# CWBudde/go-pocket-tts

Hardware: AMD Instinct MI355X
Metric: synthesized audio sec/sec (xRT) (higher is better)
Workload: dtype bf16; 1 GPU; b64_10s_bf16: 64 utterances/GPU x 125 frames (10.0 s each), 25-token prompt + 125-frame voice state, greedy (temperature 0), hipGraph-captured AR step, Mimi decode to 24 kHz PCM written to host; batch_per_gpu=64, frames=125, weights=BF16, kv=bf16, checkpoint=synthetic, shapes of tts_b6369a24 (seed 1234)

## Files before the change

### go-pocket-tts_amd/csrc/capi_hooks.cpp

```cpp
#include "capi_internal.h"
#include "launch_args.h"
#include "../../include/ptts_debug.h"
#include "scan_block.h"
#include "true_peak.h"

#include <memory>

using namespace ptts;
using namespace ptts::capi;

namespace {

template <class T> class Scoped {
    T& var_;
    T old_;
public:
    Scoped(T& var, T value) : var_(var), old_(var) { var = value; }
    ~Scoped() { var_ = old_; }
    Scoped(const Scoped&) = delete;
    Scoped& operator=(const Scoped&) = delete;
};

using Census = std::map<std::string, int64_t>;

// ... 1159 lines not shown
        if (t.ls) up(dLs.as<float>() + t.ls_off, t.ls, (size_t)D * 4);
        if (rope) { up(dCos.p, t.rope_cos, ntab * 4); up(dSin.p, t.rope_sin, ntab * 4); }
        LaunchScope launches;
        launches.run([&] {
            if (ffn) launch_mimi_ffn(fa, nullptr);
            else launch_mimi_rowlin(ra, nullptr);
        });
        PTTS_HIP(hipGetLastError());
        PTTS_HIP(hipDeviceSynchronize());
        put_str(t.launched, t.launched_cap, launches.str());
        if (ffn) down(t.out, dX.p, (size_t)t.x_elems * 4);
        else down(t.out, dY, (size_t)t.y_elems * 4);
    });
}

int ptts_mimi_layer_piece(ptts_model* h, int32_t layer, int32_t which, const float* x, int64_t rows, int32_t pos0, int32_t rows_per_seg, float* out) {
    return guard([&] {
        if (!h || !h->m) throw Error(PTTS_EINVAL, "native-safetensors runtime unavailable");
        Model& m = *h->m;
        const Desc& d = m.d;
        if (!x || !out || rows <= 0 || rows > (1 << 24)) throw Error(PTTS_EINVAL, "ptts-hip: bad rows");
        if (layer < 0 || layer >= d.mimi_layers) throw Error(PTTS_EINVAL, strfmt("ptts-hip: mimi layer %d out of range [0,%d)", layer, d.mimi_layers));
        if (which != PTTS_MIMI_PIECE_QKV && which != PTTS_MIMI_PIECE_FFN) throw Error(PTTS_EINVAL, "ptts-hip: unknown layer piece");
        if (pos0 < 0 || rows_per_seg < 0 || (int64_t)pos0 + (rows_per_seg ? rows_per_seg : rows) > ROPE_SEQ)
            throw Error(PTTS_EINVAL, strfmt("ops: rope cos/sin sequence length too small for pos=%d seq=%lld", pos0, (long long)(rows_per_seg ? rows_per_seg : rows)));
        std::lock_guard<std::mutex> lock(m.mu);
        m.use_device();
        const int C = d.mimi_dim, F = d.mimi_ffn, R = (int)rows;
        const int NO = which == PTTS_MIMI_PIECE_QKV ? 3 * C : C;
        Tmp dx((size_t)R * C * 4), dn((size_t)R * C * 4), dy((size_t)R * std::max(NO, F) * 4);
// ... 14 lines not shown
```

### go-pocket-tts_amd/csrc/ffn_fused.hip

```cpp
#include <cstdlib>
#include <type_traits>

#include "kernels.h"
#include "device_util.h"
#include "mfma_util.h"

namespace ptts {

namespace {

__device__ __forceinline__ float ff_gelu(float x) {
    const float ax = fabsf(x);
    const float t = __builtin_amdgcn_rcpf(fmaf(0.3275911f * 0.70710678118654752f, ax, 1.0f));
    float p = fmaf(1.061405429f, t, -1.453152027f);
    p = fmaf(p, t, 1.421413741f);
    p = fmaf(p, t, -0.284496736f);
    p = fmaf(p, t, 0.254829592f);
    p *= t;
    const float e = __builtin_amdgcn_exp2f(-1.4426950408889634f * 0.5f * x * x);
    const float erfa = fmaf(-p, e, 1.0f);
    const float erfs = copysignf(erfa, x);
    return 0.5f * x * (1.0f + erfs);
}

// ... 42 lines not shown
    for (int s = 0; s < 16; s++) {
        float4 o[2];
#pragma unroll
        for (int h = 0; h < 2; h++) {
            const int k = 32 * s + 16 * h + 4 * q;
            const float4 g = *reinterpret_cast<const float4*>(ln_w + k), b = *reinterpret_cast<const float4*>(ln_b + k);
            o[h].x = (v[s][h].x - mean) * rstd * g.x + b.x;
            o[h].y = (v[s][h].y - mean) * rstd * g.y + b.y;
            o[h].z = (v[s][h].z - mean) * rstd * g.z + b.z;
            o[h].w = (v[s][h].w - mean) * rstd * g.w + b.w;
        }
        split2(o[0].x, o[0].y, xh[s].u[0], xl[s].u[0]);
        split2(o[0].z, o[0].w, xh[s].u[1], xl[s].u[1]);
        split2(o[1].x, o[1].y, xh[s].u[2], xl[s].u[2]);
        split2(o[1].z, o[1].w, xh[s].u[3], xl[s].u[3]);
    }
}

template <class Piece>
__device__ __forceinline__ void ff_gemm1(const char* w1, int r16, int q, const Frag (&xh)[16], const Frag (&xl)[16], f32x4 (&acc)[2], Piece&& piece) {
    const int sw1 = (r16 >> 1) & 7;
    acc[0] = f32x4{0.f, 0.f, 0.f, 0.f};
    acc[1] = f32x4{0.f, 0.f, 0.f, 0.f};
    Frag wa[2], wb[2];
    const char* wl = w1 + r16 * 128;
    wa[0].q = *reinterpret_cast<const uint4*>(wl + ((q ^ sw1) << 4));
    wb[0].q = *reinterpret_cast<const uint4*>(wl + ((q ^ sw1) << 4) + 2048);
#pragma unroll
    for (int s = 0; s < 16; s++) {
        __builtin_amdgcn_sched_barrier(0);
// ... 104 lines not shown
#pragma unroll
            for (int t = 0; t < 8; t++) {
#pragma clang fp contract(off)
                const f32x4 y = acc2[t0 + t];
                float4 o;
                o.x = r[t].x + sc[t].x * y[0];
                o.y = r[t].y + sc[t].y * y[1];
                o.z = r[t].z + sc[t].z * y[2];
                o.w = r[t].w + sc[t].w * y[3];
                *reinterpret_cast<float4*>(orow + 16 * (t0 + t) + 4 * q) = o;
            }
        }
    }
}

__global__ __launch_bounds__(256) __attribute__((amdgpu_waves_per_eu(1, 1))) void k_mimi_rowlin(RowLinArgs a) {
    constexpr int NS = 3;
    __shared__ __attribute__((aligned(16))) char lds[NS * FF_W1B];
    const int tid = threadIdx.x, lane = tid & 63, wave = __builtin_amdgcn_readfirstlane(tid >> 6);
    const int r16 = lane & 15, q = lane >> 4;
    const int nch = a.N / FF_CH;
    const char* img = reinterpret_cast<const char*>(a.img);
    ff_dma32k(img, lds, wave, lane);
    ff_dma32k(img + (size_t)min(1, nch - 1) * FF_W1B, lds + FF_W1B, wave, lane);

    const int m0 = blockIdx.x * 64 + wave * 16;
    const int row = min(m0 + r16, a.M - 1);
    Frag xh[FF_KS], xl[FF_KS];
    ff_rows_layernorm(a.x + row_off(a.xmap, row), a.ln_w, a.ln_b, a.eps, q, xh, xl);
    float2 cs[4], sn[4];
    const bool rope = a.rope_cos != nullptr;
    {
        const int pos = a.rope_pos0 + (a.rope_rows_per_seg ? row % a.rope_rows_per_seg : row);
        const float* ct = rope ? a.rope_cos + (int64_t)pos * 32 : a.ln_w;
        const float* st = rope ? a.rope_sin + (int64_t)pos * 32 : a.ln_w;
#pragma unroll
        for (int i = 0; i < 4; i++) {
            const int jj = (32 * (i >> 1) + 16 * (i & 1) + 4 * q) >> 1;
            cs[i] = *reinterpret_cast<const float2*>(ct + jj);
            sn[i] = *reinterpret_cast<const float2*>(st + jj);
        }
    }
    float* const yrow = a.y + row_off(a.ymap, row);

    auto store_piece = [&](f32x4 (&acc)[2], int cc, auto par, int ht) {
#pragma clang fp contract(off)
        constexpr int PAR = decltype(par)::value;
        asm volatile("" : "+a"(acc[0]), "+a"(acc[1]));
        const int col = 32 * cc + 16 * ht + 4 * q;
        const bool rot = rope && 32 * cc < a.rope_cols;
        const f32x4 v = acc[ht];
        const float2 c2 = cs[2 * PAR + ht], s2 = sn[2 * PAR + ht];
        const float y0 = v[0] * c2.x - v[1] * s2.x, y1 = v[0] * s2.x + v[1] * c2.x;
        const float y2 = v[2] * c2.y - v[3] * s2.y, y3 = v[2] * s2.y + v[3] * c2.y;
        const float4 o = make_float4(rot ? y0 : v[0], rot ? y1 : v[1], rot ? y2 : v[2], rot ? y3 : v[3]);
        *reinterpret_cast<float4*>(yrow + col) = o;
    };

    asm volatile("s_waitcnt vmcnt(0)" ::: "memory");
    __syncthreads();
    f32x4 accA[2], accB[2];
    auto iter = [&](int c, auto par, auto first, f32x4 (&acc)[2], f32x4 (&prev)[2]) {
        constexpr int PAR = decltype(par)::value;
        constexpr bool FIRST = decltype(first)::value != 0;
        if constexpr (!FIRST) {
            asm volatile("s_waitcnt vmcnt(10)" ::: "memory");
            __syncthreads();
        }
        const char* const src = img + (size_t)min(c + 2, nch - 1) * FF_W1B + wave * 1024 + lane * 16;
        char* const dst = lds + ((c + 2) % NS) * FF_W1B + wave * 1024;
        ff_gemm1(lds + (c % NS) * FF_W1B, r16, q, xh, xl, acc, [&](int s) {
            if ((s & 1) == 0) lds_dma1k(src + (s >> 1) * 4096, dst + (s >> 1) * 4096);
            if constexpr (!FIRST) {
                if (s == 5) store_piece(prev, c - 1, std::integral_constant<int, 1 - PAR>{}, 0);
                if (s == 11) store_piece(prev, c - 1, std::integral_constant<int, 1 - PAR>{}, 1);
            }
        });
    };
    using ic0 = std::integral_constant<int, 0>;
    using ic1 = std::integral_constant<int, 1>;
    iter(0, ic0{}, ic1{}, accA, accB);
    iter(1, ic1{}, ic0{}, accB, accA);
    for (int c = 2; c < nch; c += 2) {
        iter(c, ic0{}, ic0{}, accA, accB);
        iter(c + 1, ic1{}, ic0{}, accB, accA);
    }
    store_piece(accB, nch - 1, std::integral_constant<int, 1>{}, 0);
    store_piece(accB, nch - 1, std::integral_constant<int, 1>{}, 1);
}

bool mimi_rowlin_supported(const RowLinArgs& a) {
    return a.img && a.K == FF_D && a.N >= 64 && a.N % 64 == 0 && a.M > 0 && aligned16(a.x) && a.xmap.ld % 4 == 0 && a.xmap.batch_stride % 4 == 0 && aligned16(a.y) &&
           a.ymap.ld % 4 == 0 && a.ymap.batch_stride % 4 == 0 && aligned16(a.img) && a.ln_w && a.ln_b && aligned16(a.ln_w) && aligned16(a.ln_b) &&
           (!a.rope_cos || (a.rope_sin && a.rope_cols % 64 == 0 && a.rope_cols <= a.N && (reinterpret_cast<uintptr_t>(a.rope_cos) & 7) == 0 && (reinterpret_cast<uintptr_t>(a.rope_sin) & 7) == 0));
}

void launch_mimi_rowlin(const RowLinArgs& a, hipStream_t stream) {
    note_launch(a.rope_cos ? "k_mimi_rowlin+rope" : "k_mimi_rowlin");
    hipLaunchKernelGGL(k_mimi_rowlin, dim3((unsigned)((a.M + 63) / 64)), dim3(256), 0, stream, a);
}

bool mimi_ffn_supported(const FfnArgs& a) {
    return a.img && a.D == FF_D && a.F >= FF_CH && a.F % FF_CH == 0 && a.M > 0 && aligned16(a.x) && a.xmap.ld % 4 == 0 && a.xmap.batch_stride % 4 == 0 &&
           aligned16(a.img) && a.ln_w && a.ln_b && aligned16(a.ln_w) && aligned16(a.ln_b) && (!a.ls || aligned16(a.ls));
}

void launch_mimi_ffn(const FfnArgs& a, hipStream_t stream) {
    note_launch("k_mimi_ffn");
    const dim3 grid((unsigned)((a.M + 63) / 64));
    hipLaunchKernelGGL(k_mimi_ffn<0>, grid, dim3(256), 0, stream, a);
}

}
```

### go-pocket-tts_amd/csrc/kernels.h

```cpp
#pragma once

#include <hip/hip_runtime.h>
#include <atomic>
#include <cstddef>
#include <cstdint>
#include <map>
#include <string>
#include <vector>

#include "deesser.h"
#include "limiter.h"
#include "pitch.h"
#include "tempo.h"
#include "trim.h"

namespace ptts {

struct RowMap {
    int64_t ld = 0;
    int64_t rows_per_batch = 0;
    int64_t batch_stride = 0;
};

enum AOp : int { AOP_NONE = 0, AOP_ELU = 1 };
// ... 398 lines not shown

struct FfnArgs {
    float* x = nullptr; RowMap xmap;
    const float* ln_w = nullptr; const float* ln_b = nullptr; float eps = 1e-5f;
    const void* img = nullptr;
    const float* ls = nullptr;
    int M = 0, D = 0, F = 0;
};
struct RowLinArgs {
    const float* x = nullptr; RowMap xmap;
    const float* ln_w = nullptr; const float* ln_b = nullptr; float eps = 1e-5f;
    const void* img = nullptr;
    float* y = nullptr; RowMap ymap;
    const float* rope_cos = nullptr; const float* rope_sin = nullptr; int rope_cols = 0, rope_pos0 = 0, rope_rows_per_seg = 0;
    int M = 0, N = 0, K = 0;
};
bool mimi_rowlin_supported(const RowLinArgs& a);
void launch_mimi_rowlin(const RowLinArgs& a, hipStream_t stream);
bool mimi_ffn_supported(const FfnArgs& a);
void launch_mimi_ffn(const FfnArgs& a, hipStream_t stream);

constexpr int FC_MAX_DEPTH = 8;
struct FlowClusterArgs {
    const float* fx_in = nullptr; float* fx_out = nullptr;
    const float* ada = nullptr; int64_t ldmod = 0;
    int rows = 0, depth = 0;
    float eps[FC_MAX_DEPTH] = {};
    const float* ln_w[FC_MAX_DEPTH] = {}; const float* ln_b[FC_MAX_DEPTH] = {};
    const void* w0[FC_MAX_DEPTH] = {}; const float* b0[FC_MAX_DEPTH] = {};
    const void* w2[FC_MAX_DEPTH] = {}; const float* b2[FC_MAX_DEPTH] = {};
    unsigned long long* xbuf = nullptr;
    unsigned long long* stamps = nullptr;
    int inject = 0;
// ... 68 lines not shown
```

### go-pocket-tts_amd/csrc/mimi_decode.cpp

```cpp
#include "launch_args.h"

#include <algorithm>

namespace ptts {

void mimi_setup(Model& m, MimiWs& w, int B, int T) {
    const Desc& d = m.d;
    w.B = B; w.T = T;
    const int C = d.mimi_dim, S = d.up_stride, T1 = T * S, F = d.mimi_ffn;
    w.P0 = d.init_k - 1;
    w.Ls[0] = T1; w.Ps[0] = 1;
    for (int j = 0; j < 3; j++) {
        w.Ls[j + 1] = w.Ls[j] * d.strides[j];
        int need_next = j < 2 ? 1 : d.final_k - 1;
        w.Ps[j + 1] = std::max(d.rb_k1[j] - 1, need_next);
    }
    size_t n_xp = (size_t)B * (1 + T) * C, n_up = (size_t)B * (w.P0 + T1) * C;
    size_t n_n1 = (size_t)B * T1 * C, n_qkv = (size_t)B * T1 * 3 * C, n_ff = (size_t)B * T1 * F;
    size_t n_c[4], n_h[3];
    for (int j = 0; j < 4; j++) n_c[j] = (size_t)B * (w.Ps[j] + w.Ls[j]) * d.sea_ch[j];
    for (int j = 0; j < 3; j++) n_h[j] = (size_t)B * ((d.rb_k2[j] - 1) + w.Ls[j + 1]) * d.sea_hidden[j];
    size_t total = n_xp + n_up + n_n1 + n_qkv * d.mimi_layers + n_n1 + n_ff + n_c[0] + 2 * (n_c[1] + n_c[2] + n_c[3]) + n_h[0] + n_h[1] + n_h[2];
    DevBuf& wsb = m.work(WORK_DECODER, total * sizeof(float));
    float* p = wsb.as<float>();
// ... 39 lines not shown
        ra.M = R; ra.N = 3 * C; ra.K = C;
        if (mimi_rowlin_supported(ra)) { launch_mimi_rowlin(ra, s); return; }
    }
    launch_layernorm(mkln(m, x, xmap, L.n1, n1, C, R), s);
    GemmArgs gq = mk(m, n1, flat(C), L.in_proj, qkv, qmap, R);
    gq.rope_cos = m.at<float>(d.rope_cos); gq.rope_sin = m.at<float>(d.rope_sin);
    gq.rope_cols = 2 * C; gq.rope_hd = d.mimi_hd; gq.rope_pos0 = pos0; gq.rope_rows_per_seg = rows_per_seg;
    if (!launch_gemm_rope(gq, s)) {
        gq.rope_cos = gq.rope_sin = nullptr;
        launch_gemm(gq, s);
        launch_rope_rows(qkv, qmap, 0, d.mimi_heads, d.mimi_hd, nullptr, pos0, rows_per_seg, R, m.at<float>(d.rope_cos), m.at<float>(d.rope_sin), s);
        launch_rope_rows(qkv, qmap, C, d.mimi_heads, d.mimi_hd, nullptr, pos0, rows_per_seg, R, m.at<float>(d.rope_cos), m.at<float>(d.rope_sin), s);
    }
}

void mimi_layer_ffn(Model& m, int l, float* x, RowMap xmap, int R, float* n1, float* ffb, hipStream_t s) {
    mimi_layer_ffn(m, m.d.ml[l], x, xmap, R, n1, ffb, s);
}
void mimi_layer_ffn(Model& m, const Desc::ML& L, float* x, RowMap xmap, int R, float* n1, float* ffb, hipStream_t s) {
    const Desc& d = m.d;
    const int C = d.mimi_dim, F = d.mimi_ffn;
    if (L.ffn_img != NONE) {
        FfnArgs fa;
        fa.x = x; fa.xmap = xmap;
        fa.ln_w = m.at<float>(L.n2.w); fa.ln_b = m.at<float>(L.n2.b); fa.eps = L.n2.eps;
        fa.img = m.at<uint8_t>(L.ffn_img);
        fa.ls = m.at<float>(L.ls2);
        fa.M = R; fa.D = C; fa.F = F;
        if (mimi_ffn_supported(fa)) { launch_mimi_ffn(fa, s); return; }
    }
// ... 13 lines not shown
    const int B = w.B, T = w.T, C = d.mimi_dim, S = d.up_stride, T1 = T * S, P0 = w.P0;
    if (f1 <= f0) return;
    if (!w.zeroed) mimi_zero_history(m, w, s);
    const int nf = f1 - f0;
    launch_projector(lat, lat_bstride, m.at<float>(d.proj_w), m.at<float>(d.proj_b), B, T, f0, f1, d.ldim, C, w.xp, s);
    if (mimi_latent) launch_btc_to_bct(w.xp, 1, B, C, T, mimi_latent, s);
    launch_upsample_depthwise(w.xp, m.at<float>(d.up_w0), m.at<float>(d.up_w1), nullptr, B, T, f0, f1, C, S, w.up, P0, s);
    const int t0 = f0 * S, CT = nf * S, R = B * CT;
    const int64_t up_bs = (int64_t)(P0 + T1) * C;
    float* upx = w.up + (size_t)(P0 + t0) * C;
    const RowMap upm = seg(C, CT, up_bs);
    float* n1 = w.n1;
    float* attn = w.attn;
    float* ffb = w.ff;
    for (int l = 0; l < d.mimi_layers; l++) {
        const auto& L = d.ml[l];
        float* qkv = w.qkv[l];
        float* qkvx = qkv + (size_t)t0 * 3 * C;
        const RowMap qm = seg(3 * C, CT, (int64_t)T1 * 3 * C);
        mimi_layer_qkv(m, l, upx, upm, R, qkvx, qm, t0, CT, n1, s);
        launch_attention(attn_dense_args(qkv, 3 * C, C, B, T1, t0, CT, d.mimi_heads, d.mimi_hd, d.mimi_ctx, attn, C), s);
        GemmArgs go = mk(m, attn, flat(C), L.out_proj, upx, upm, R);
        go.R = upx; go.epi = L.ls1 != NONE ? EPI_SCALE_RESADD : EPI_RESADD; go.scale = m.at<float>(L.ls1);
        launch_gemm(go, s);
        mimi_layer_ffn(m, l, upx, upm, R, n1, ffb, s);
    }
    if (xformer_out)
        PTTS_HIP(hipMemcpy2DAsync(xformer_out + (size_t)t0 * C, (size_t)T1 * C * sizeof(float), upx, (size_t)up_bs * sizeof(float), (size_t)CT * C * sizeof(float),
                                  (size_t)B, hipMemcpyDeviceToDevice, s));
    int r0 = t0, rn = CT;
    {
        const int ch = d.sea_ch[0];
        GemmArgs g = mk(m, w.up + (size_t)r0 * C, seg(C, rn, up_bs), d.init_conv, w.c0 + (size_t)(w.Ps[0] + r0) * ch,
                        seg(ch, rn, (int64_t)(w.Ps[0] + w.Ls[0]) * ch), B * rn);
        g.epi = EPI_ELU;
        if (C % 64 == 0 && d.init_conv.in == d.init_k * C) { g.win_taps = d.init_k; g.win_c = C; }
        launch_gemm(g, s);
    }
    bool final_done = false;
// ... 91 lines not shown
```

### go-pocket-tts_amd/csrc/runtime.cpp

```cpp
#include "launch_args.h"

#include <chrono>

#include <algorithm>

namespace ptts {

static thread_local UploadArena* tl_upload = nullptr;
static void arena_open(UploadArena& a) {
    if (!a.base && hipHostMalloc((void**)&a.base, (size_t)1 << 20, hipHostMallocDefault) == hipSuccess) a.cap = (size_t)1 << 20;
    else if (!a.base) (void)hipGetLastError();
    a.off = 0;
    tl_upload = &a;
}
UploadScope::UploadScope(UploadArena& a, hipStream_t s) {
    (void)hipStreamSynchronize(s);
    arena_open(a);
}
UploadScope::UploadScope(UploadArena& a, hipEvent_t last_use) {
    if (last_use) (void)hipEventSynchronize(last_use);
    arena_open(a);
}
UploadScope::~UploadScope() { tl_upload = nullptr; }
void h2d(void* dst, const void* src, size_t bytes, hipStream_t s) {
// ... 14 lines not shown
    if (!bytes) return;
    PTTS_HIP(hipMemcpyAsync(dst, src, bytes, hipMemcpyDeviceToHost, s));
    PTTS_HIP(hipStreamSynchronize(s));
}

Model::~Model() {
    if (upload.base) (void)hipHostFree(upload.base);
    for (hipEvent_t e : prof.ev) (void)hipEventDestroy(e);
    for (hipEvent_t e : prof.phase) if (e) (void)hipEventDestroy(e);
    for (hipEvent_t e : events) (void)hipEventDestroy(e);
    if (stream2) (void)hipStreamDestroy(stream2);

    cached_batch.reset();
    tcomb.clear();
    for (DevBuf& w : ws) w.release();
    if (own_arena && arena) (void)hipFree(arena);
    if (stream) (void)hipStreamDestroy(stream);
}

static std::unique_ptr<Model> model_on(const Desc& d, const ptts_opts& opts, int device) {
    std::unique_ptr<Model> m(new Model());
    m->d = d;
    m->opts = opts;
    m->opts.device = m->device = device;
    m->noise_state = (uint64_t)std::chrono::system_clock::now().time_since_epoch().count() ^ (uint64_t)(uintptr_t)m.get();
    return m;
}
static void open_streams(Model& m) {
    m.use_device();
    int lo = 0, hi = 0;
// ... 12 lines not shown
    open_streams(*m);
    if (device_arena) {
        m->arena = reinterpret_cast<uint8_t*>(device_arena);
    } else {
        void* p = nullptr;
        PTTS_HIP(hipMalloc(&p, m->d.total_bytes));
        m->arena = reinterpret_cast<uint8_t*>(p);
        m->own_arena = true;
        fill = 1;
    }
    if (fill) {
        std::vector<uint8_t> host(m->d.total_bytes, 0);
        plan_fill(*plan, host.data());
        PTTS_HIP(hipMemcpy(m->arena, host.data(), host.size(), hipMemcpyHostToDevice));
    }
    return m.release();
}

Model* model_share(Model& base) {
    std::unique_ptr<Model> m = model_on(base.d, base.opts, base.device);
    open_streams(*m);
    m->arena = base.arena;
    m->own_arena = false;
    return m.release();
}

Model* model_replicate(Model& base, int device) {
    int ndev = 0;
    if (hipGetDeviceCount(&ndev) != hipSuccess || ndev <= 0) throw Error(PTTS_ENODEVICE, "ptts-hip: no HIP device available (this library has no CPU fallback)");
    if (device < 0 || device >= ndev) throw Error(PTTS_ENODEVICE, strfmt("ptts-hip: device %d out of range (%d visible)", device, ndev));
    std::unique_ptr<Model> m = model_on(base.d, base.opts, device);
    {
        std::lock_guard<std::mutex> lock(base.mu);
        base.use_device();
        PTTS_HIP(hipStreamSynchronize(base.stream));
    }
    open_streams(*m);
    void* p = nullptr;
    PTTS_HIP(hipMalloc(&p, m->d.total_bytes));
    m->arena = reinterpret_cast<uint8_t*>(p);
    m->own_arena = true;
    if (device != base.device) {
        int can = 0;
        if (hipDeviceCanAccessPeer(&can, device, base.device) == hipSuccess && can) {
            const hipError_t e = hipDeviceEnablePeerAccess(base.device, 0);
            if (e != hipSuccess && e != hipErrorPeerAccessAlreadyEnabled) (void)hipGetLastError();
            else if (e == hipErrorPeerAccessAlreadyEnabled) (void)hipGetLastError();
        }
    }
    PTTS_HIP(hipMemcpyPeer(m->arena, device, base.arena, base.device, m->d.total_bytes));
    PTTS_HIP(hipDeviceSynchronize());
    return m.release();
}

void profile_read(Model& m, ptts_profile* out) {
    PTTS_HIP(hipStreamSynchronize(m.stream));
    std::memset(out, 0, sizeof *out);
    double ms = 0;
    for (size_t i = 0; i + 1 < m.prof.used; i += 2) {
        float t = 0;
        PTTS_HIP(hipEventElapsedTime(&t, m.prof.ev[i], m.prof.ev[i + 1]));
        ms += t;
    }
    out->launches = m.prof.launches;
    out->total_ms = ms;
    out->algorithmic_bytes = m.prof.bytes;
// ... 107 lines not shown
```

### go-pocket-tts_amd/csrc/runtime.h

```cpp
#pragma once

#include <atomic>
#include <functional>
#include <type_traits>

#include "kernels.h"
#include "model.h"
#include "row_ring.h"
#include "dsp_spec.h"
#include "host_rows.h"
#include "join.h"

namespace ptts {

struct DevBuf {
    void* p = nullptr;
    size_t n = 0;
    DevBuf() = default;
    DevBuf(const DevBuf&) = delete;
    DevBuf& operator=(const DevBuf&) = delete;
    ~DevBuf() { release(); }
    void release() {
        if (p) (void)hipFree(p);
        p = nullptr;
// ... 126 lines not shown
    size_t cap = 0, off = 0;
};

struct Model {
    Desc d;
    ptts_opts opts;
    uint8_t* arena = nullptr;
    bool own_arena = false;
    int device = 0;
    hipStream_t stream = nullptr;
    hipStream_t stream2 = nullptr;
    std::vector<hipEvent_t> events;
    std::mutex mu;
    std::map<int, std::unique_ptr<DevBuf>> tcomb;
    DevBuf ws[kWorkSlots];
    std::unique_ptr<Batch> cached_batch;
    Prof prof;
    std::map<std::pair<int, int>, std::unique_ptr<RateFilter>> rate_filters;
    RowRing<ResampleRow> rs_ring;
    RowRing<CmpRow, kCmpMaxDesigns * kCmpScanBytes> cmp_ring;
    RowRing<LimRow, kLimMaxDesigns * kLimScanBytes> lim_ring;
    RowRing<DeRow, kDeMaxDesigns * kDeScanBytes> de_ring;
    RowRing<JoinRow> join_ring;
    RowRing<JoinGainRow> join_gain_ring;
    RowRing<TrimRow, kTrimMaxDesigns * kTrimScanBytes> trim_ring;
    RowRing<TempoRow, kTempoMaxDesigns * kTempoScanBytes> tempo_ring;
    RowRing<PitchRow, kPitchMaxDesigns * kPitchScanBytes> pitch_ring;
    std::unique_ptr<UploadedTable> pitch_image;
    RowRing<FormantRow> formant_ring;
    std::unique_ptr<UploadedTable> formant_tables;
// ... 105 lines not shown

struct MimiWs {
    int B = 0, T = 0, P0 = 0;
    int Ls[4] = {0, 0, 0, 0}, Ps[4] = {0, 0, 0, 0};
    float *xp = nullptr, *up = nullptr, *n1 = nullptr, *qkv[MAX_LAYERS] = {nullptr}, *attn = nullptr, *ff = nullptr, *c0 = nullptr;
    float *u[3] = {nullptr, nullptr, nullptr}, *uo[3] = {nullptr, nullptr, nullptr}, *h[3] = {nullptr, nullptr, nullptr};
    bool zeroed = false;
};
constexpr int kMimiGroup = 64;
void mimi_setup(Model& m, MimiWs& w, int B, int T);
void mimi_range(Model& m, MimiWs& w, const float* lat, int64_t lat_bstride, int f0, int f1, float* pcm, float* mimi_latent, hipStream_t s,
                const PcmRow* pcm_rows = nullptr, bool* rows_used = nullptr, float* xformer_out = nullptr);

void mimi_layer_qkv(Model& m, int layer, const float* x, RowMap xmap, int R, float* qkv, RowMap qmap, int pos0, int rows_per_seg, float* n1, hipStream_t s);
void mimi_layer_ffn(Model& m, int layer, float* x, RowMap xmap, int R, float* n1, float* ffb, hipStream_t s);
void mimi_layer_qkv(Model& m, const Desc::ML& L, const float* x, RowMap xmap, int R, float* qkv, RowMap qmap, int pos0, int rows_per_seg, float* n1, hipStream_t s);
void mimi_layer_ffn(Model& m, const Desc::ML& L, float* x, RowMap xmap, int R, float* n1, float* ffb, hipStream_t s);

constexpr int kEncStages = 10;
int64_t mimi_encode_max_frames(const Desc& d);
void mimi_encode(Model& m, const float* const* pcm, const int64_t* n_samples, int n_clips, float* const* latent_out, float* const* stages = nullptr,
                 const int32_t* rates = nullptr);
int64_t mimi_encode_clip(Model& m, const float* pcm, int64_t n_samples, float* lat_dev, float* const* stages = nullptr, int rate = kNativeRate);
int64_t mimi_encode_samples(int64_t n_samples, int rate);
void require_encoder(const Desc& d);
void mimi_encode_stage_shapes(const Desc& d, int64_t n_samples, int64_t* shapes );
Model* model_open(Plan* plan, void* device_arena, int fill);
void profile_read(Model& m, ptts_profile* out);
Batch* batch_new(Model& m, int n_slots, int cap, int max_steps);
void batch_reset(Batch& b);
// ... 192 lines not shown
```

### go-pocket-tts_amd/runtime.py

```python
from __future__ import annotations

import ctypes as C
import os
import subprocess
import sys
from dataclasses import dataclass, field
from typing import Callable, Optional, Sequence

import numpy as np

_HERE = os.path.dirname(os.path.abspath(__file__))
LIB_PATH = os.environ.get("PTTS_LIB_PATH") or os.path.join(_HERE, "libptts_hip.so")

PTTS_OK, PTTS_EINVAL, PTTS_EIO, PTTS_EFORMAT, PTTS_ENODEVICE, PTTS_ECANCELLED, PTTS_ENOMEM = range(7)
WEIGHTS_F32, WEIGHTS_BF16, WEIGHTS_INT8 = 0, 1, 2
KV_F32, KV_BF16 = 0, 1
PCM_F32, PCM_S16, PCM_ULAW, PCM_ALAW = 0, 1, 2, 3
_PCM_DTYPES = {PCM_F32: "<f4", PCM_S16: "<i2", PCM_ULAW: "|u1", PCM_ALAW: "|u1"}

_FP = C.POINTER(C.c_float)
_IP = C.POINTER(C.c_int64)
_DP = C.POINTER(C.c_double)
_I32P = C.POINTER(C.c_int32)
_STEP_CB = C.CFUNCTYPE(None, C.c_void_p, C.c_int32, C.c_int32)
# ... 218 lines not shown
    "ptts_join_parts_length", "ptts_join_parts", "ptts_join_parts_rows", "ptts_join_parts_stream_ready", "ptts_generate_joined_parts",
    "ptts_trim_plan", "ptts_trim_apply", "ptts_trim_rows", "ptts_dsp_ext_set_trim",
    "ptts_tempo_length", "ptts_tempo_plan", "ptts_tempo_apply", "ptts_tempo_rows", "ptts_dsp_ext_set_tempo",
    "ptts_pitch_speed", "ptts_pitch_resample_length", "ptts_pitch_resample", "ptts_pitch_length", "ptts_pitch_apply", "ptts_pitch_table",
    "ptts_pitch_rows", "ptts_dsp_ext_set_pitch",
    "ptts_formant_frames", "ptts_formant_analyse", "ptts_formant_whiten", "ptts_formant_shape", "ptts_formant_apply", "ptts_formant_rows",
    "ptts_dsp_ext_set_formant",
    ]
HOOK_SYMBOLS = [
    "ptts_decode_stages", "ptts_mimi_layer_piece", "ptts_debug_last_attention_kernel", "ptts_debug_launch_counts", "ptts_debug_flow_cluster_inject",
    "ptts_debug_time_skinny", "ptts_debug_skinny_stamps", "ptts_debug_gemm", "ptts_debug_step_stamps", "ptts_debug_tall_linear",
    "ptts_debug_encode_stages", "ptts_debug_resample_launches", "ptts_debug_dsp_blocked_host",
    "ptts_debug_loudness_energies", "ptts_debug_kweighting", "ptts_debug_step_linear", "ptts_debug_true_peak_taps", "ptts_debug_true_peak_oversample",
    "ptts_debug_dsp_opts_error", "ptts_debug_resblock", "ptts_debug_resblock_plan", "ptts_debug_seanet_pack", "ptts_debug_plan_seanet_frags",
    "ptts_debug_gemm_rows", "ptts_debug_attn_step", "ptts_debug_attn_step_rounds", "ptts_debug_attn_window", "ptts_debug_flow_cluster",
    "ptts_debug_mimi_fused", "ptts_debug_mimi_pack", "ptts_debug_dsp_windows", "ptts_debug_step_edge",
]


def build(force: bool = False) -> str:
    args = ["make", "-s", "-C", _HERE, "-j8"]
    if force:
        args.append("-B")
    subprocess.check_call(args)
    return LIB_PATH


def lib():
    global _lib
    if _lib is None:
        if not os.path.exists(LIB_PATH):
# ... 1469 lines not shown
    a.y_ld, a.y_rows_per_batch, a.y_batch_stride, a.y_off = (int(v) for v in ymap)
    a.x, a.ln_w, a.ln_b, a.w1, a.w2, a.ls = ptr(x_buf), ptr(ln_w), ptr(ln_b), ptr(w1), ptr(w2), ptr(ls)
    if rope is not None:
        cos, sin = (None if t is None else _f32(t) for t in rope)
        a.rope_cos, a.rope_sin = ptr(cos), ptr(sin)
        a.n_pos = (cos if cos is not None else sin).shape[0]
        a.rope_cols, a.pos0, a.rows_per_seg = int(rope_cols), int(pos0), int(rows_per_seg)
    out = np.empty(x_buf.size if int(kind) == 0 else max(int(y_elems), 1), np.float32)
    a.out = ptr(out)
    name = C.create_string_buffer(512)
    a.launched, a.launched_cap = C.cast(name, C.c_char_p), 512
    _check(hooks().ptts_debug_mimi_fused(C.byref(a)))
    return {"out": out, "launched": _census_dict(name)}


def debug_mimi_pack(kind, w1, w2=None):
    w1 = _f32(w1)
    n = w1.shape[0]
    if w1.ndim != 2 or w1.shape[1] != 512 or (kind == 0 and (w2 is None or tuple(np.shape(w2)) != (512, n))):
        raise ValueError("w1 is [n, 512], w2 [512, n]")
    w2 = None if kind != 0 else _f32(w2)
    dst = np.empty(n * (1024 if kind == 0 else 512), np.uint16)
    H = hooks()
    H.ptts_debug_mimi_pack.argtypes = [C.c_int32, _FP, _FP, C.c_int32, C.c_void_p]
    _check(H.ptts_debug_mimi_pack(int(kind), _fp(w1), C.cast(None, _FP) if w2 is None else _fp(w2), n, dst.ctypes.data_as(C.c_void_p)))
    return dst.reshape((n // 32, 2, 16384) if kind == 0 else (n // 32, 16384))


class _ResblockArgs(C.Structure):
    _fields_ = ([(n, C.c_int32) for n in ("B", "L", "t0", "t1", "C", "H", "pad", "slack", "w_bf16", "final_conv", "form", "grid", "fuse_up", "x_pad", "x_L", "x_slack")] +
# ... 878 lines not shown
```

### include/ptts_debug.h

```cpp
#ifndef PTTS_DEBUG_H
#define PTTS_DEBUG_H

#include "ptts.h"

#ifdef __cplusplus
extern "C" {
#endif

#define PTTS_MIMI_PIECE_QKV 0
#define PTTS_MIMI_PIECE_FFN 1
int  ptts_mimi_layer_piece(ptts_model* m, int32_t layer, int32_t which, const float* x, int64_t rows, int32_t pos0, int32_t rows_per_seg, float* out);

int  ptts_decode_stages(ptts_model* m, const float* latents, int32_t n_utt, int32_t frames,
                        float* pcm, float* mimi_latent, float* transformer_out);

int  ptts_debug_encode_stages(ptts_model* m, const float* pcm, int64_t n_samples, float* const* stages, int64_t* shapes);

int ptts_debug_time_skinny(int32_t M, int32_t N, int32_t K, int32_t w_bf16, int32_t splitk, int32_t fuse_ln, int32_t iters, float* avg_us);
int ptts_debug_skinny_stamps(int32_t M, int32_t N, int32_t K, int32_t w_bf16, int32_t splitk, int32_t fuse_ln, uint64_t* out ,
                             int32_t max_blocks, int32_t* n_blocks);
int ptts_debug_step_stamps(ptts_batch* b, int32_t lsd_steps, uint64_t* out , int64_t cap_blocks, int32_t* desc ,
                           int32_t cap_desc, int32_t* n_desc);
int ptts_debug_gemm(int32_t M, int32_t N, int32_t K, int32_t w_bf16, int32_t variant, int32_t epi, int32_t iters, float* avg_us,
                    float* maxdiff);
// ... 115 lines not shown
    char* launched;
} ptts_flow_cluster_args;
int ptts_debug_flow_cluster(const ptts_flow_cluster_args* a);

typedef struct ptts_mimi_fused_args {
    int32_t kind, M, D, F, n_pos, rope_cols, pos0, rows_per_seg, ls_off, reserved;
    float eps, reserved_f;
    int64_t x_elems, x_ld, x_rows_per_batch, x_batch_stride, x_off, y_elems, y_ld, y_rows_per_batch, y_batch_stride, y_off, launched_cap;
    const float *x, *ln_w, *ln_b, *w1, *w2, *ls, *rope_cos, *rope_sin;
    float* out;
    char* launched;
} ptts_mimi_fused_args;
int ptts_debug_mimi_fused(const ptts_mimi_fused_args* a);
int ptts_debug_mimi_pack(int32_t kind, const float* w1, const float* w2, int32_t n, uint16_t* dst);

int64_t ptts_debug_dsp_opts_error(const ptts_dsp_opts* opts, char* out, int64_t cap);
int ptts_debug_true_peak_taps(float* out , int32_t* L, int32_t* K, int32_t* dlo);
int ptts_debug_true_peak_oversample(const float* samples, int64_t n, float* y );

#ifdef __cplusplus
}
#endif
#endif
```

Measured before the change: 12890 x real-time.

## Route Mimi attention out-projection through pre-packed row-linear kernel with residual epilogue

Adds a residual-add variant of the k_mimi_rowlin kernel, templated on the epilogue. The Mimi transformer's 512x512 attention output projection now uses it instead of the generic GEMM. Weight images in the swizzled LDS-DMA layout are packed once at model load, and the kernel skips layernorm and rope, applying the layer-scale and residual add in its epilogue. The aim is to replace a generic GEMM with the tuned, pipelined weight-streaming kernel. The cost is extra device memory for the packed images, plus a load-time pack and sync.

After: 12850 x real-time. No clear change (-0.3%).

```diff
diff --git a/go-pocket-tts_amd/csrc/capi_hooks.cpp b/go-pocket-tts_amd/csrc/capi_hooks.cpp
--- a/go-pocket-tts_amd/csrc/capi_hooks.cpp
+++ b/go-pocket-tts_amd/csrc/capi_hooks.cpp
@@ -1197,6 +1197,48 @@
     });
 }
 
+int ptts_debug_mimi_out(const ptts_mimi_out_args* pa) {
+    return guard([&] {
+        if (!pa) throw Error(PTTS_EINVAL, "ptts_debug_mimi_out: null argument");
+        const ptts_mimi_out_args& t = *pa;
+        constexpr int D = 512;
+        if (!t.attn || !t.r || !t.w || !t.out || t.M < 1 || t.M > (1 << 20) || t.attn_rows < t.M || t.x_elems < 1 || t.x_ld < 1 || t.x_rows_per_batch < 0 ||
+            t.x_rows_per_batch > INT32_MAX || t.x_batch_stride < 0 || t.x_off < 0 || (t.w_bf16 | t.path | t.in_place) & ~1)
+            throw Error(PTTS_EINVAL, "ptts_debug_mimi_out: bad arguments");
+        if (t.x_ld % 4 || t.x_batch_stride % 4 || t.x_off % 4) throw Error(PTTS_EINVAL, "ptts_debug_mimi_out: x_ld, x_batch_stride and x_off must be multiples of 4");
+        const RowMap xmap{t.x_ld, t.x_rows_per_batch, t.x_batch_stride};
+        check_rows("ptts_debug_mimi_out", "r", t.M, t.x_elems, xmap, t.x_off, D, true);
+        require_device();
+        Stage st;
+        const size_t nw = (size_t)D * D;
+        GemmArgs go;
+        const uint8_t* img = nullptr;
+        if (t.w_bf16) {
+            std::vector<uint16_t> w16(nw);
+            for (size_t i = 0; i < nw; i++) w16[i] = f32_to_bf16_rne(t.w[i]);
+            go.W = st.in(w16.data(), nw);
+            if (t.path == 0) {
+                uint16_t* dimg = st.out<uint16_t>(nw);
+                launch_w1_image_pack(go.W, dimg, D, nullptr);
+                img = reinterpret_cast<const uint8_t*>(dimg);
+            }
+        } else go.W = st.in(t.w, nw);
+        go.w_bf16 = t.w_bf16; go.ldw = D;
+        go.A = st.in(t.attn, (size_t)t.attn_rows * D); go.amap = flat(D);
+        float* const dR = st.in(t.r, (size_t)t.x_elems);
+        float* const dY = t.in_place ? dR : st.out((size_t)t.x_elems);
+        go.R = dR + t.x_off; go.C = dY + t.x_off; go.cmap = xmap;
+        go.scale = st.in(t.ls, (size_t)D); go.epi = t.ls ? EPI_SCALE_RESADD : EPI_RESADD;
+        go.M = t.M; go.N = D; go.K = D;
+        LaunchScope launches;
+        launches.run([&] { mimi_out_launch(go, img, nullptr); });
+        PTTS_HIP(hipGetLastError());
+        PTTS_HIP(hipDeviceSynchronize());
+        put_str(t.launched, t.launched_cap, launches.str());
+        down(t.out, dY, (size_t)t.x_elems * 4);
+    });
+}
+
 int ptts_mimi_layer_piece(ptts_model* h, int32_t layer, int32_t which, const float* x, int64_t rows, int32_t pos0, int32_t rows_per_seg, float* out) {
     return guard([&] {
         if (!h || !h->m) throw Error(PTTS_EINVAL, "native-safetensors runtime unavailable");
diff --git a/go-pocket-tts_amd/csrc/ffn_fused.hip b/go-pocket-tts_amd/csrc/ffn_fused.hip
--- a/go-pocket-tts_amd/csrc/ffn_fused.hip
+++ b/go-pocket-tts_amd/csrc/ffn_fused.hip
@@ -80,6 +80,22 @@
         split2(o[0].z, o[0].w, xh[s].u[1], xl[s].u[1]);
         split2(o[1].x, o[1].y, xh[s].u[2], xl[s].u[2]);
         split2(o[1].z, o[1].w, xh[s].u[3], xl[s].u[3]);
+    }
+}
+
+__device__ __forceinline__ void ff_rows_split(const float* xrow, int q, Frag (&xh)[16], Frag (&xl)[16]) {
+    float4 v[16][2];
+#pragma unroll
+    for (int s = 0; s < 16; s++) {
+        v[s][0] = *reinterpret_cast<const float4*>(xrow + 32 * s + 4 * q);
+        v[s][1] = *reinterpret_cast<const float4*>(xrow + 32 * s + 16 + 4 * q);
+    }
+#pragma unroll
+    for (int s = 0; s < 16; s++) {
+        split2(v[s][0].x, v[s][0].y, xh[s].u[0], xl[s].u[0]);
+        split2(v[s][0].z, v[s][0].w, xh[s].u[1], xl[s].u[1]);
+        split2(v[s][1].x, v[s][1].y, xh[s].u[2], xl[s].u[2]);
+        split2(v[s][1].z, v[s][1].w, xh[s].u[3], xl[s].u[3]);
     }
 }
 
@@ -214,23 +230,42 @@
     }
 }
 
+template <int EPI>
 __global__ __launch_bounds__(256) __attribute__((amdgpu_waves_per_eu(1, 1))) void k_mimi_rowlin(RowLinArgs a) {
+    constexpr bool RES = EPI == ROWLIN_RESADD;
     constexpr int NS = 3;
-    __shared__ __attribute__((aligned(16))) char lds[NS * FF_W1B];
+    __shared__ __attribute__((aligned(16))) char lds[NS * FF_W1B + (RES ? FF_D * 4 : 0)];
     const int tid = threadIdx.x, lane = tid & 63, wave = __builtin_amdgcn_readfirstlane(tid >> 6);
     const int r16 = lane & 15, q = lane >> 4;
-    const int nch = a.N / FF_CH;
+    const int nch = RES ? FF_D / FF_CH : a.N / FF_CH;
     const char* img = reinterpret_cast<const char*>(a.img);
     ff_dma32k(img, lds, wave, lane);
     ff_dma32k(img + (size_t)min(1, nch - 1) * FF_W1B, lds + FF_W1B, wave, lane);
 
     const int m0 = blockIdx.x * 64 + wave * 16;
     const int row = min(m0 + r16, a.M - 1);
+    const bool live = m0 + r16 < a.M;
+    const float* const xrow = a.x + row_off(a.xmap, row);
+    float* const yrow = a.y + row_off(a.ymap, row);
     Frag xh[FF_KS], xl[FF_KS];
-    ff_rows_layernorm(a.x + row_off(a.xmap, row), a.ln_w, a.ln_b, a.eps, q, xh, xl);
+    float4 rr[RES ? FF_OT : 1];
+    const float* const lsl = reinterpret_cast<const float*>(lds + NS * FF_W1B);
+    if constexpr (RES) {
+        float2 sv = make_float2(1.f, 1.f);
+        if (a.ls) sv = *reinterpret_cast<const float2*>(a.ls + 2 * tid);
+        *reinterpret_cast<float2*>(lds + NS * FF_W1B + 8 * tid) = sv;
+        const float* const rrow = live ? a.res + row_off(a.ymap, row) : xrow;
+#pragma unroll
+        for (int t = 0; t < FF_OT; t++) rr[t] = *reinterpret_cast<const float4*>(rrow + 16 * t + 4 * q);
+        ff_rows_split(xrow, q, xh, xl);
+#pragma unroll
+        for (int t = 0; t < FF_OT; t++) asm volatile("" : "+v"(rr[t].x), "+v"(rr[t].y), "+v"(rr[t].z), "+v"(rr[t].w));
+    } else {
+        ff_rows_layernorm(xrow, a.ln_w, a.ln_b, a.eps, q, xh, xl);
+    }
     float2 cs[4], sn[4];
-    const bool rope = a.rope_cos != nullptr;
-    {
+    const bool rope = !RES && a.rope_cos != nullptr;
+    if constexpr (!RES) {
         const int pos = a.rope_pos0 + (a.rope_rows_per_seg ? row % a.rope_rows_per_seg : row);
         const float* ct = rope ? a.rope_cos + (int64_t)pos * 32 : a.ln_w;
         const float* st = rope ? a.rope_sin + (int64_t)pos * 32 : a.ln_w;
@@ -241,13 +276,24 @@
             sn[i] = *reinterpret_cast<const float2*>(st + jj);
         }
     }
-    float* const yrow = a.y + row_off(a.ymap, row);
 
     auto store_piece = [&](f32x4 (&acc)[2], int cc, auto par, int ht) {
 #pragma clang fp contract(off)
         constexpr int PAR = decltype(par)::value;
         asm volatile("" : "+a"(acc[0]), "+a"(acc[1]));
         const int col = 32 * cc + 16 * ht + 4 * q;
+        if constexpr (RES) {
+            const f32x4 v = acc[ht];
+            const float4 sc = *reinterpret_cast<const float4*>(lsl + col);
+            const float4 r = rr[2 * cc + ht];
+            float4 o;
+            o.x = r.x + sc.x * v[0];
+            o.y = r.y + sc.y * v[1];
+            o.z = r.z + sc.z * v[2];
+            o.w = r.w + sc.w * v[3];
+            if (live) *reinterpret_cast<float4*>(yrow + col) = o;
+            return;
+        }
         const bool rot = rope && 32 * cc < a.rope_cols;
         const f32x4 v = acc[ht];
         const float2 c2 = cs[2 * PAR + ht], s2 = sn[2 * PAR + ht];
@@ -264,7 +310,8 @@
         constexpr int PAR = decltype(par)::value;
         constexpr bool FIRST = decltype(first)::value != 0;
         if constexpr (!FIRST) {
-            asm volatile("s_waitcnt vmcnt(10)" ::: "memory");
+            if constexpr (RES) asm volatile("s_waitcnt vmcnt(8)" ::: "memory");
+            else asm volatile("s_waitcnt vmcnt(10)" ::: "memory");
             __syncthreads();
         }
         const char* const src = img + (size_t)min(c + 2, nch - 1) * FF_W1B + wave * 1024 + lane * 16;
@@ -281,23 +328,55 @@
     using ic1 = std::integral_constant<int, 1>;
     iter(0, ic0{}, ic1{}, accA, accB);
     iter(1, ic1{}, ic0{}, accB, accA);
-    for (int c = 2; c < nch; c += 2) {
-        iter(c, ic0{}, ic0{}, accA, accB);
-        iter(c + 1, ic1{}, ic0{}, accB, accA);
+    if constexpr (RES) {
+#pragma unroll
+        for (int c = 2; c < FF_D / FF_CH; c += 2) {
+            iter(c, ic0{}, ic0{}, accA, accB);
+            iter(c + 1, ic1{}, ic0{}, accB, accA);
+        }
+    } else {
+        for (int c = 2; c < nch; c += 2) {
+            iter(c, ic0{}, ic0{}, accA, accB);
+            iter(c + 1, ic1{}, ic0{}, accB, accA);
+        }
     }
     store_piece(accB, nch - 1, std::integral_constant<int, 1>{}, 0);
     store_piece(accB, nch - 1, std::integral_constant<int, 1>{}, 1);
 }
 
+__global__ __launch_bounds__(256) void k_w1_image_pack(const uint16_t* __restrict__ w, uint16_t* __restrict__ img, int n_pieces) {
+    const int p = blockIdx.x * 256 + threadIdx.x;
+    if (p >= n_pieces) return;
+    const int pos = p & 7, h = (p >> 3) & 31, j = (p >> 8) & 7, c = p >> 11;
+    const int sgq = pos ^ ((h >> 1) & 7), s = 2 * j + (sgq >> 2), qq = sgq & 3;
+    const uint16_t* src = w + (size_t)(32 * c + h) * FF_D + 32 * s + 4 * qq;
+    const uint2 lo = *reinterpret_cast<const uint2*>(src), hi = *reinterpret_cast<const uint2*>(src + 16);
+    *reinterpret_cast<uint4*>(img + (size_t)p * 8) = make_uint4(lo.x, lo.y, hi.x, hi.y);
+}
+
+void launch_w1_image_pack(const void* w_bf16, void* img, int N, hipStream_t stream) {
+    const int n_pieces = N / 32 * 2048;
+    hipLaunchKernelGGL(k_w1_image_pack, dim3((unsigned)((n_pieces + 255) / 256)), dim3(256), 0, stream, reinterpret_cast<const uint16_t*>(w_bf16), reinterpret_cast<uint16_t*>(img),
+                       n_pieces);
+}
+
 bool mimi_rowlin_supported(const RowLinArgs& a) {
-    return a.img && a.K == FF_D && a.N >= 64 && a.N % 64 == 0 && a.M > 0 && aligned16(a.x) && a.xmap.ld % 4 == 0 && a.xmap.batch_stride % 4 == 0 && aligned16(a.y) &&
-           a.ymap.ld % 4 == 0 && a.ymap.batch_stride % 4 == 0 && aligned16(a.img) && a.ln_w && a.ln_b && aligned16(a.ln_w) && aligned16(a.ln_b) &&
+    const bool rows_ok = a.img && a.K == FF_D && a.M > 0 && aligned16(a.x) && a.xmap.ld % 4 == 0 && a.xmap.batch_stride % 4 == 0 && aligned16(a.y) && a.ymap.ld % 4 == 0 &&
+                         a.ymap.batch_stride % 4 == 0 && aligned16(a.img);
+    if (a.epi == ROWLIN_RESADD) return rows_ok && a.N == FF_D && a.res && aligned16(a.res) && !a.rope_cos && !a.rope_sin && (!a.ls || aligned16(a.ls));
+    return a.epi == ROWLIN_ROPE && rows_ok && a.N >= 64 && a.N % 64 == 0 && a.ln_w && a.ln_b && aligned16(a.ln_w) && aligned16(a.ln_b) && !a.ls &&
            (!a.rope_cos || (a.rope_sin && a.rope_cols % 64 == 0 && a.rope_cols <= a.N && (reinterpret_cast<uintptr_t>(a.rope_cos) & 7) == 0 && (reinterpret_cast<uintptr_t>(a.rope_sin) & 7) == 0));
 }
 
 void launch_mimi_rowlin(const RowLinArgs& a, hipStream_t stream) {
+    const dim3 grid((unsigned)((a.M + 63) / 64));
+    if (a.epi == ROWLIN_RESADD) {
+        note_launch("k_mimi_rowlin+resadd");
+        hipLaunchKernelGGL(k_mimi_rowlin<ROWLIN_RESADD>, grid, dim3(256), 0, stream, a);
+        return;
+    }
     note_launch(a.rope_cos ? "k_mimi_rowlin+rope" : "k_mimi_rowlin");
-    hipLaunchKernelGGL(k_mimi_rowlin, dim3((unsigned)((a.M + 63) / 64)), dim3(256), 0, stream, a);
+    hipLaunchKernelGGL(k_mimi_rowlin<ROWLIN_ROPE>, grid, dim3(256), 0, stream, a);
 }
 
 bool mimi_ffn_supported(const FfnArgs& a) {
diff --git a/go-pocket-tts_amd/csrc/kernels.h b/go-pocket-tts_amd/csrc/kernels.h
--- a/go-pocket-tts_amd/csrc/kernels.h
+++ b/go-pocket-tts_amd/csrc/kernels.h
@@ -436,9 +436,13 @@
     float* y = nullptr; RowMap ymap;
     const float* rope_cos = nullptr; const float* rope_sin = nullptr; int rope_cols = 0, rope_pos0 = 0, rope_rows_per_seg = 0;
     int M = 0, N = 0, K = 0;
-};
+    int epi = 0;
+    const float* res = nullptr; const float* ls = nullptr;
+};
+enum { ROWLIN_ROPE = 0, ROWLIN_RESADD = 1 };
 bool mimi_rowlin_supported(const RowLinArgs& a);
 void launch_mimi_rowlin(const RowLinArgs& a, hipStream_t stream);
+void launch_w1_image_pack(const void* w_bf16, void* img, int N, hipStream_t stream);
 bool mimi_ffn_supported(const FfnArgs& a);
 void launch_mimi_ffn(const FfnArgs& a, hipStream_t stream);
 
diff --git a/go-pocket-tts_amd/csrc/mimi_decode.cpp b/go-pocket-tts_amd/csrc/mimi_decode.cpp
--- a/go-pocket-tts_amd/csrc/mimi_decode.cpp
+++ b/go-pocket-tts_amd/csrc/mimi_decode.cpp
@@ -77,6 +77,46 @@
     }
 }
 
+void mimi_layer_out(Model& m, int l, const float* attn, float* x, RowMap xmap, int R, hipStream_t s) {
+    const Desc::ML& L = m.d.ml[l];
+    GemmArgs go = mk(m, attn, flat(m.d.mimi_dim), L.out_proj, x, xmap, R);
+    go.R = x; go.epi = L.ls1 != NONE ? EPI_SCALE_RESADD : EPI_RESADD; go.scale = m.at<float>(L.ls1);
+    mimi_out_launch(go, m.out_img[l], s);
+}
+void mimi_out_launch(const GemmArgs& go, const uint8_t* img, hipStream_t s) {
+    if (img && (go.epi == EPI_SCALE_RESADD || go.epi == EPI_RESADD) && !go.bias && go.aop == AOP_NONE) {
+        RowLinArgs ra;
+        ra.epi = ROWLIN_RESADD;
+        ra.x = go.A; ra.xmap = go.amap;
+        ra.img = img;
+        ra.res = go.R; ra.y = go.C; ra.ymap = go.cmap;
+        ra.ls = go.epi == EPI_SCALE_RESADD ? go.scale : nullptr;
+        ra.M = go.M; ra.N = go.N; ra.K = go.K;
+        if (mimi_rowlin_supported(ra)) { launch_mimi_rowlin(ra, s); return; }
+    }
+    launch_gemm(go, s);
+}
+
+void mimi_out_images(Model& m) {
+    const Desc& d = m.d;
+    auto takes = [&](const Lin& o) { return o.bf16 && o.w != NONE && o.in == 512 && o.out == 512 && o.b == NONE && d.mimi_dim == 512; };
+    int n = 0;
+    for (int l = 0; l < d.mimi_layers; l++) n += takes(d.ml[l].out_proj) ? 1 : 0;
+    if (!n) return;
+    const size_t per = (size_t)512 * 512 * 2;
+    m.use_device();
+    m.out_img_buf.ensure(per * n);
+    int i = 0;
+    for (int l = 0; l < d.mimi_layers; l++) {
+        if (!takes(d.ml[l].out_proj)) continue;
+        uint8_t* img = m.out_img_buf.as<uint8_t>() + per * i++;
+        launch_w1_image_pack(m.arena + d.ml[l].out_proj.w, img, 512, m.stream);
+        m.out_img[l] = img;
+    }
+    PTTS_HIP(hipGetLastError());
+    PTTS_HIP(hipStreamSynchronize(m.stream));
+}
+
 void mimi_layer_ffn(Model& m, int l, float* x, RowMap xmap, int R, float* n1, float* ffb, hipStream_t s) {
     mimi_layer_ffn(m, m.d.ml[l], x, xmap, R, n1, ffb, s);
 }
@@ -120,15 +160,12 @@
     float* attn = w.attn;
     float* ffb = w.ff;
     for (int l = 0; l < d.mimi_layers; l++) {
-        const auto& L = d.ml[l];
         float* qkv = w.qkv[l];
         float* qkvx = qkv + (size_t)t0 * 3 * C;
         const RowMap qm = seg(3 * C, CT, (int64_t)T1 * 3 * C);
         mimi_layer_qkv(m, l, upx, upm, R, qkvx, qm, t0, CT, n1, s);
         launch_attention(attn_dense_args(qkv, 3 * C, C, B, T1, t0, CT, d.mimi_heads, d.mimi_hd, d.mimi_ctx, attn, C), s);
-        GemmArgs go = mk(m, attn, flat(C), L.out_proj, upx, upm, R);
-        go.R = upx; go.epi = L.ls1 != NONE ? EPI_SCALE_RESADD : EPI_RESADD; go.scale = m.at<float>(L.ls1);
-        launch_gemm(go, s);
+        mimi_layer_out(m, l, attn, upx, upm, R, s);
         mimi_layer_ffn(m, l, upx, upm, R, n1, ffb, s);
     }
     if (xformer_out)
diff --git a/go-pocket-tts_amd/csrc/runtime.cpp b/go-pocket-tts_amd/csrc/runtime.cpp
--- a/go-pocket-tts_amd/csrc/runtime.cpp
+++ b/go-pocket-tts_amd/csrc/runtime.cpp
@@ -52,6 +52,7 @@
     cached_batch.reset();
     tcomb.clear();
     for (DevBuf& w : ws) w.release();
+    out_img_buf.release();
     if (own_arena && arena) (void)hipFree(arena);
     if (stream) (void)hipStreamDestroy(stream);
 }
@@ -94,6 +95,7 @@
         plan_fill(*plan, host.data());
         PTTS_HIP(hipMemcpy(m->arena, host.data(), host.size(), hipMemcpyHostToDevice));
     }
+    mimi_out_images(*m);
     return m.release();
 }
 
@@ -102,6 +104,7 @@
     open_streams(*m);
     m->arena = base.arena;
     m->own_arena = false;
+    std::copy(std::begin(base.out_img), std::end(base.out_img), std::begin(m->out_img));
     return m.release();
 }
 
@@ -130,6 +133,7 @@
     }
     PTTS_HIP(hipMemcpyPeer(m->arena, device, base.arena, base.device, m->d.total_bytes));
     PTTS_HIP(hipDeviceSynchronize());
+    mimi_out_images(*m);
     return m.release();
 }
 
diff --git a/go-pocket-tts_amd/csrc/runtime.h b/go-pocket-tts_amd/csrc/runtime.h
--- a/go-pocket-tts_amd/csrc/runtime.h
+++ b/go-pocket-tts_amd/csrc/runtime.h
@@ -164,6 +164,8 @@
     std::mutex mu;
     std::map<int, std::unique_ptr<DevBuf>> tcomb;
     DevBuf ws[kWorkSlots];
+    DevBuf out_img_buf;
+    const uint8_t* out_img[MAX_LAYERS] = {};
     std::unique_ptr<Batch> cached_batch;
     Prof prof;
     std::map<std::pair<int, int>, std::unique_ptr<RateFilter>> rate_filters;
@@ -299,6 +301,9 @@
 
 void mimi_layer_qkv(Model& m, int layer, const float* x, RowMap xmap, int R, float* qkv, RowMap qmap, int pos0, int rows_per_seg, float* n1, hipStream_t s);
 void mimi_layer_ffn(Model& m, int layer, float* x, RowMap xmap, int R, float* n1, float* ffb, hipStream_t s);
+void mimi_layer_out(Model& m, int layer, const float* attn, float* x, RowMap xmap, int R, hipStream_t s);
+void mimi_out_launch(const GemmArgs& go, const uint8_t* img, hipStream_t s);
+void mimi_out_images(Model& m);
 void mimi_layer_qkv(Model& m, const Desc::ML& L, const float* x, RowMap xmap, int R, float* qkv, RowMap qmap, int pos0, int rows_per_seg, float* n1, hipStream_t s);
 void mimi_layer_ffn(Model& m, const Desc::ML& L, float* x, RowMap xmap, int R, float* n1, float* ffb, hipStream_t s);
 
diff --git a/go-pocket-tts_amd/runtime.py b/go-pocket-tts_amd/runtime.py
--- a/go-pocket-tts_amd/runtime.py
+++ b/go-pocket-tts_amd/runtime.py
@@ -256,7 +256,7 @@
     "ptts_debug_loudness_energies", "ptts_debug_kweighting", "ptts_debug_step_linear", "ptts_debug_true_peak_taps", "ptts_debug_true_peak_oversample",
     "ptts_debug_dsp_opts_error", "ptts_debug_resblock", "ptts_debug_resblock_plan", "ptts_debug_seanet_pack", "ptts_debug_plan_seanet_frags",
     "ptts_debug_gemm_rows", "ptts_debug_attn_step", "ptts_debug_attn_step_rounds", "ptts_debug_attn_window", "ptts_debug_flow_cluster",
-    "ptts_debug_mimi_fused", "ptts_debug_mimi_pack", "ptts_debug_dsp_windows", "ptts_debug_step_edge",
+    "ptts_debug_mimi_fused", "ptts_debug_mimi_pack", "ptts_debug_dsp_windows", "ptts_debug_step_edge", "ptts_debug_mimi_out",
 ]
 
 
@@ -1756,6 +1756,33 @@
     return {"out": out, "launched": _census_dict(name)}
 
 
+class _MimiOutArgs(C.Structure):
+    _fields_ = ([(n, C.c_int32) for n in ("M", "attn_rows", "w_bf16", "path", "in_place", "reserved")] +
+                [(n, C.c_int64) for n in ("x_elems", "x_ld", "x_rows_per_batch", "x_batch_stride", "x_off", "launched_cap")] +
+                [(n, _FP) for n in ("attn", "r", "w", "ls", "out")] + [("launched", C.c_char_p)])
+
+
+MIMI_OUT_AUTO, MIMI_OUT_GEMM = 0, 1
+
+
+def debug_mimi_out(attn, r_buf, M, w, *, xmap, ls=None, w_bf16=True, path=MIMI_OUT_AUTO, in_place=True):
+    attn, r_buf, w = _f32(attn), _f32(r_buf).reshape(-1), _f32(w)
+    if attn.ndim != 2 or attn.shape[1] != 512 or w.shape != (512, 512):
+        raise ValueError("attn is [rows, 512], w [512, 512]")
+    a, keep = _MimiOutArgs(), _Keep()
+    ptr = keep.f32
+    a.M, a.attn_rows, a.w_bf16, a.path, a.in_place = int(M), attn.shape[0], int(bool(w_bf16)), int(path), int(bool(in_place))
+    a.x_elems = r_buf.size
+    a.x_ld, a.x_rows_per_batch, a.x_batch_stride, a.x_off = (int(v) for v in xmap)
+    a.attn, a.r, a.w, a.ls = ptr(attn), ptr(r_buf), ptr(w), ptr(ls)
+    out = np.empty(r_buf.size, np.float32)
+    a.out = ptr(out)
+    name = C.create_string_buffer(512)
+    a.launched, a.launched_cap = C.cast(name, C.c_char_p), 512
+    _check(hooks().ptts_debug_mimi_out(C.byref(a)))
+    return {"out": out, "launched": _census_dict(name)}
+
+
 def debug_mimi_pack(kind, w1, w2=None):
     w1 = _f32(w1)
     n = w1.shape[0]
diff --git a/include/ptts_debug.h b/include/ptts_debug.h
--- a/include/ptts_debug.h
+++ b/include/ptts_debug.h
@@ -153,6 +153,15 @@
 int ptts_debug_mimi_fused(const ptts_mimi_fused_args* a);
 int ptts_debug_mimi_pack(int32_t kind, const float* w1, const float* w2, int32_t n, uint16_t* dst);
 
+typedef struct ptts_mimi_out_args {
+    int32_t M, attn_rows, w_bf16, path, in_place, reserved;
+    int64_t x_elems, x_ld, x_rows_per_batch, x_batch_stride, x_off, launched_cap;
+    const float *attn, *r, *w, *ls;
+    float* out;
+    char* launched;
+} ptts_mimi_out_args;
+int ptts_debug_mimi_out(const ptts_mimi_out_args* a);
+
 int64_t ptts_debug_dsp_opts_error(const ptts_dsp_opts* opts, char* out, int64_t cap);
 int ptts_debug_true_peak_taps(float* out , int32_t* L, int32_t* K, int32_t* dlo);
 int ptts_debug_true_peak_oversample(const float* samples, int64_t n, float* y );
```
